# rhofield/rho-tts

Hardware: AMD Instinct MI355X
Metric: audio-sec/wall-sec (RTF) Qwen3-TTS-1.7B batch=32 (higher is better)
Workload: dtype bf16; 1 GPU; Qwen3-TTS-1.7B bf16, batch 32/GPU, 30-s reference clone, 10-word sentences (44 frames each), sampling=top-k 50 T 0.9, seeded synthetic weights; value counts delivered (post-processed) audio; global_batch=32, parallelism=dp1

## Files before the change

### rho_tts_amd/csrc/attention.hip

```cpp
#include "kernels.h"

namespace {

typedef __attribute__((ext_vector_type(4))) unsigned u4_t;

template <int D, int REP, bool FUSED, int NW, bool LO = false>
__global__ __launch_bounds__(NW * 64) void k_attention(const float* __restrict__ q, int heads, int kv_heads,
                                                   const int32_t* __restrict__ row_slot, const int32_t* __restrict__ row_pos,
                                                   int pos_add, int window, bf16_t* __restrict__ kc, bf16_t* __restrict__ vc,
                                                   int max_pos, bf16_t* __restrict__ out, const float* __restrict__ qw,
                                                   const float* __restrict__ kw, float eps, const float* __restrict__ cosT,
                                                   const float* __restrict__ sinT, const int32_t* __restrict__ frame_ptr, int out_tiled, int prefix_slot,
                                                   int prefix_len, const bf16_t* __restrict__ kc_lo, const bf16_t* __restrict__ vc_lo,
                                                   float* __restrict__ out_f32, int slot_base, int pair_n) {
    constexpr int LPP = D / 8;
    constexpr int PPW = 64 / LPP;
    constexpr int U = 4;
    __shared__ float sh[NW][REP][LPP][10];
    __shared__ float sh_q[FUSED ? REP : 1][FUSED ? D : 1];
    __shared__ __attribute__((aligned(16))) bf16_t sh_kv[2][FUSED ? D : 8];
    __shared__ __attribute__((aligned(16))) bf16_t sh_kv2[2][FUSED ? D : 8];

    const int kh = blockIdx.x, row = blockIdx.y;
    const int lane = threadIdx.x & 63, w = threadIdx.x >> 6;
    const int sub = lane % LPP, pg = lane / LPP;
    constexpr int half = D / 2;
    const int width = (heads + 2 * kv_heads) * D;
    const bool act = lane < half;
    float pa = 0.f, pb = 0.f, pwa = 0.f, pwb = 0.f, pc = 0.f, psn = 0.f;
    const int l0 = act ? lane : 0;
    if (FUSED) {
        const int v0 = w < REP + 2 ? w : REP + 1;
        const int col0 = v0 < REP ? (kh * REP + v0) * D : (v0 == REP ? (heads + kh) * D : (heads + kv_heads + kh) * D);
        const float* src = q + (int64_t)row * width + col0;
        pa = src[l0];
        pb = src[l0 + half];
        const float* nw = v0 < REP ? qw : kw;
        const float* nwp = nw ? nw : src;
        pwa = nwp[l0];
        pwb = nwp[l0 + half];
    }
    const int slot = row_slot ? row_slot[row] : slot_base + row;
    const int hi = (row_pos ? row_pos[row] : 0) + pos_add + (frame_ptr ? *frame_ptr : 0);
    if (FUSED) { pc = cosT[(int64_t)hi * half + l0]; psn = sinT[(int64_t)hi * half + l0]; }
    int lo = 0;
    if (window > 0 && hi - window + 1 > 0) lo = hi - window + 1;
    const float scale = rsqrtf((float)D);
    const bool partner = FUSED && pair_n > 0 && row >= pair_n && hi >= 1;
    const int64_t base = ((int64_t)slot * kv_heads + kh) * max_pos;
    const bf16_t* kb = kc + base * D + sub * 8;
    const bf16_t* vb = vc + base * D + sub * 8;
    const int64_t pdelta = prefix_slot >= 0 ? (((int64_t)prefix_slot - slot) * kv_heads * max_pos) * D : 0;
    constexpr int STEP = NW * PPW;
    u4_t kk[U], vv[U];
    u4_t kl[LO ? U : 1], vl[LO ? U : 1];
    auto load_batch = [&](int p0, int last) {
#pragma unroll
        for (int u = 0; u < U; ++u) {
            const int p = p0 + u * STEP;
            int pc = p <= last ? p : last;
            if (pc < 0) pc = 0;
            const int64_t po = (int64_t)pc * D + (pc < prefix_len ? pdelta : 0);
            kk[u] = *reinterpret_cast<const u4_t*>(kb + po);
            vv[u] = *reinterpret_cast<const u4_t*>(vb + po);
            if (LO) {
                kl[LO ? u : 0] = *reinterpret_cast<const u4_t*>(kc_lo + base * D + sub * 8 + po);
                vl[LO ? u : 0] = *reinterpret_cast<const u4_t*>(vc_lo + base * D + sub * 8 + po);
            }
        }
    };
    const int p_first = lo + w * PPW + pg;
    constexpr int RPL = (D * 2 >= 128) ? 1 : 128 / (D * 2);
    const int pre_last = (hi / RPL) * RPL - 1;
    constexpr bool PRE = FUSED && REP <= 2;
    if (PRE) load_batch(p_first, pre_last);

    if (FUSED) {
        for (int vec = w; vec < REP + 2 + (partner ? 2 : 0); vec += NW) {
            const bool mate = vec >= REP + 2;
            const bool is_q = vec < REP, is_k = vec == REP || vec == REP + 2;
            const int col0 = is_q ? (kh * REP + vec) * D : (is_k ? (heads + kh) * D : (heads + kv_heads + kh) * D);
            const bool first = vec == w && !mate;
            const int vrow = mate ? row - pair_n : row, vpos = mate ? hi - 1 : hi;
            float a = pa, b = pb;
            if (!first && act) { a = q[(int64_t)vrow * width + col0 + lane]; b = q[(int64_t)vrow * width + col0 + lane + half]; }
            if (is_q || is_k) {
                const float* nw = is_q ? qw : kw;
                if (nw) {
                    float wa = pwa, wb = pwb;
                    if (!first && act) { wa = nw[lane]; wb = nw[lane + half]; }
                    const float ss = wave_sum_rows_f32(act ? a * a + b * b : 0.f);
                    const float inv = rsqrtf(ss / (float)D + eps);
                    if (act) { a = wa * (a * inv); b = wb * (b * inv); }
                }
                if (act) {
                    float c = pc, s = psn;
                    if (!first) { c = cosT[(int64_t)vpos * half + lane]; s = sinT[(int64_t)vpos * half + lane]; }
                    const float ra = a * c - b * s, rb = b * c + a * s;
                    a = ra; b = rb;
                }
            }
            if (act) {
                if (is_q) { sh_q[FUSED ? vec : 0][FUSED ? lane : 0] = a; sh_q[FUSED ? vec : 0][FUSED ? lane + half : 0] = b; }
                else if (mate) {
                    sh_kv2[is_k ? 0 : 1][FUSED ? lane : 0] = f32_to_bf16(a);
                    sh_kv2[is_k ? 0 : 1][FUSED ? lane + half : 0] = f32_to_bf16(b);
                } else {
                    bf16_t* o = (is_k ? kc : vc) + (((int64_t)slot * kv_heads + kh) * max_pos + hi) * D;
                    const bf16_t ra = f32_to_bf16(a), rb = f32_to_bf16(b);
                    o[lane] = ra;
                    o[lane + half] = rb;
                    sh_kv[is_k ? 0 : 1][FUSED ? lane : 0] = ra;
                    sh_kv[is_k ? 0 : 1][FUSED ? lane + half : 0] = rb;
                }
            }
        }
        __syncthreads();
    }

    float qr[REP][8];
#pragma unroll
    for (int r = 0; r < REP; ++r) {
#pragma unroll
        for (int j = 0; j < 8; ++j) {
            if (FUSED) qr[r][j] = sh_q[FUSED ? r : 0][FUSED ? sub * 8 + j : 0] * scale;
            else qr[r][j] = q[((int64_t)row * heads + kh * REP + r) * D + sub * 8 + j] * scale;
        }
    }
    float m[REP], l[REP], acc[REP][8];
#pragma unroll
    for (int r = 0; r < REP; ++r) {
        m[r] = -1e30f;
        l[r] = 0.f;
#pragma unroll
        for (int j = 0; j < 8; ++j) acc[r][j] = 0.f;
    }
    for (int p0 = p_first; p0 <= hi; p0 += STEP * U) {
        if (PRE && p0 == p_first) {
#pragma unroll
            for (int u = 0; u < U; ++u) {
                const int p = p0 + u * STEP;
                if (p == hi) {
                    kk[u] = *reinterpret_cast<const u4_t*>(&sh_kv[0][FUSED ? sub * 8 : 0]);
                    vv[u] = *reinterpret_cast<const u4_t*>(&sh_kv[1][FUSED ? sub * 8 : 0]);
                } else if (partner && p == hi - 1) {
                    kk[u] = *reinterpret_cast<const u4_t*>(&sh_kv2[0][FUSED ? sub * 8 : 0]);
                    vv[u] = *reinterpret_cast<const u4_t*>(&sh_kv2[1][FUSED ? sub * 8 : 0]);
                } else if (p > pre_last && p < hi) {
                    const int64_t po = (int64_t)p * D + (p < prefix_len ? pdelta : 0);
                    kk[u] = *reinterpret_cast<const u4_t*>(kb + po);
                    vv[u] = *reinterpret_cast<const u4_t*>(vb + po);
                }
            }
        } else {
            load_batch(p0, hi);
        }
#pragma unroll
        for (int u = 0; u < U; ++u) {
            const int p = p0 + u * NW * PPW;
            float kf[8], vf[8];
#pragma unroll
            for (int j = 0; j < 4; ++j) {
                kf[2 * j] = __uint_as_float(kk[u][j] << 16);
                kf[2 * j + 1] = __uint_as_float(kk[u][j] & 0xffff0000u);
                vf[2 * j] = __uint_as_float(vv[u][j] << 16);
                vf[2 * j + 1] = __uint_as_float(vv[u][j] & 0xffff0000u);
                if (LO) {
                    kf[2 * j] += __uint_as_float(kl[LO ? u : 0][j] << 16);
                    kf[2 * j + 1] += __uint_as_float(kl[LO ? u : 0][j] & 0xffff0000u);
                    vf[2 * j] += __uint_as_float(vl[LO ? u : 0][j] << 16);
                    vf[2 * j + 1] += __uint_as_float(vl[LO ? u : 0][j] & 0xffff0000u);
                }
            }
#pragma unroll
            for (int r = 0; r < REP; ++r) {
                float s = 0.f;
#pragma unroll
                for (int j = 0; j < 8; ++j) s += qr[r][j] * kf[j];
                s = group_sum_f32<LPP>(s);
                if (p <= hi) {
                    const float mn = fmaxf(m[r], s);
                    const float corr = __expf(m[r] - mn), pe = __expf(s - mn);
                    l[r] = l[r] * corr + pe;
#pragma unroll
                    for (int j = 0; j < 8; ++j) acc[r][j] = acc[r][j] * corr + pe * vf[j];
                    m[r] = mn;
                }
            }
        }
    }
#pragma unroll
    for (int r = 0; r < REP; ++r) {
#pragma unroll
        for (int o = LPP; o < 64; o <<= 1) {
            const float m2 = __shfl_xor(m[r], o, 64), l2 = __shfl_xor(l[r], o, 64);
            const float mn = fmaxf(m[r], m2);
            const float c1 = __expf(m[r] - mn), c2 = __expf(m2 - mn);
            l[r] = l[r] * c1 + l2 * c2;
#pragma unroll
            for (int j = 0; j < 8; ++j) acc[r][j] = acc[r][j] * c1 + __shfl_xor(acc[r][j], o, 64) * c2;
            m[r] = mn;
        }
        if (pg == 0) {
            sh[w][r][sub][0] = m[r];
            sh[w][r][sub][1] = l[r];
#pragma unroll
            for (int j = 0; j < 8; ++j) sh[w][r][sub][2 + j] = acc[r][j];
        }
    }
    __syncthreads();
    for (int t = threadIdx.x; t < REP * LPP * 8; t += NW * 64) {
        const int j = t & 7, sb = (t >> 3) % LPP, r = t / (8 * LPP);
        float mn = -1e30f;
#pragma unroll
        for (int ww = 0; ww < NW; ++ww) mn = fmaxf(mn, sh[ww][r][sb][0]);
        float lt = 0.f, at = 0.f;
#pragma unroll
        for (int ww = 0; ww < NW; ++ww) {
            const float c = __expf(sh[ww][r][sb][0] - mn);
            lt += sh[ww][r][sb][1] * c;
            at += sh[ww][r][sb][2 + j] * c;
        }
        const int kcol = (kh * REP + r) * D + sb * 8 + j;
        const int64_t oo = out_tiled ? tile_off(row, kcol, heads * D) : (int64_t)row * heads * D + kcol;
        if (LO) out_f32[(int64_t)row * heads * D + kcol] = lt > 0.f ? at / lt : 0.f;
        else out[oo] = f32_to_bf16(lt > 0.f ? at / lt : 0.f);
    }
}

struct FusedArgs { const float *qw, *kw, *cosT, *sinT; float eps; const int32_t* frame_ptr; int out_tiled; int prefix_slot, prefix_len;
                   const bf16_t *kc_lo = nullptr, *vc_lo = nullptr; float* out_f32 = nullptr; int slot_base = 0; int pair_n = 0; };

template <int D, bool FUSED, int NW, bool LO = false>
int dispatch_rep(rt_ctx* ctx, int rep, dim3 grid, const float* q, int heads, int kv_heads, const int32_t* rs, const int32_t* rp,
                 int pos_add, int window, bf16_t* kc, bf16_t* vc, int max_pos, bf16_t* out, const FusedArgs& f) {
    switch (rep) {
        case 1: hipLaunchKernelGGL((k_attention<D, 1, FUSED, NW, LO>), grid, dim3(NW * 64), 0, ctx->stream, q, heads, kv_heads, rs, rp, pos_add, window, kc, vc, max_pos, out, f.qw, f.kw, f.eps, f.cosT, f.sinT, f.frame_ptr, f.out_tiled, f.prefix_slot, f.prefix_len, f.kc_lo, f.vc_lo, f.out_f32, f.slot_base, f.pair_n); break;
        case 2: hipLaunchKernelGGL((k_attention<D, 2, FUSED, NW, LO>), grid, dim3(NW * 64), 0, ctx->stream, q, heads, kv_heads, rs, rp, pos_add, window, kc, vc, max_pos, out, f.qw, f.kw, f.eps, f.cosT, f.sinT, f.frame_ptr, f.out_tiled, f.prefix_slot, f.prefix_len, f.kc_lo, f.vc_lo, f.out_f32, f.slot_base, f.pair_n); break;
        case 4: hipLaunchKernelGGL((k_attention<D, 4, FUSED, NW, LO>), grid, dim3(NW * 64), 0, ctx->stream, q, heads, kv_heads, rs, rp, pos_add, window, kc, vc, max_pos, out, f.qw, f.kw, f.eps, f.cosT, f.sinT, f.frame_ptr, f.out_tiled, f.prefix_slot, f.prefix_len, f.kc_lo, f.vc_lo, f.out_f32, f.slot_base, f.pair_n); break;
        default: return rt_fail(ctx, RT_ERR_UNSUPPORTED, "attention: heads/kv_heads = %d unsupported (1, 2, 4)", rep);
    }
    RT_HIP(ctx, hipGetLastError());
    return RT_OK;
}

template <bool FUSED>
int attention_any(rt_ctx* ctx, const float* q, int M, int heads, int kv_heads, int head_dim, const int32_t* row_slot, const int32_t* row_pos,
                  int pos_add, int window, const KvCache& kv, int layer, bf16_t* out, const FusedArgs& f0) {
    if (M <= 0) return RT_OK;
    FusedArgs f = f0;
    f.prefix_slot = kv.prefix_slot;
    f.prefix_len = kv.prefix_slot >= 0 ? kv.prefix_len : 0;
    if (heads % kv_heads) return rt_fail(ctx, RT_ERR_INVALID, "attention: heads %d not a multiple of kv_heads %d", heads, kv_heads);
    const int rep = heads / kv_heads;
    bf16_t* kc = kv.k + layer * kv.layer_stride();
    bf16_t* vc = kv.v + layer * kv.layer_stride();
    dim3 grid(kv_heads, M);
    if (kv.k_lo) {
        if (FUSED || !f.out_f32 || !kv.v_lo) return rt_fail(ctx, RT_ERR_INVALID, "attention: hi/lo cache needs the unfused form and a float32 output");
        f.kc_lo = kv.k_lo + layer * kv.layer_stride();
        f.vc_lo = kv.v_lo + layer * kv.layer_stride();
        switch (head_dim) {
            case 32: return dispatch_rep<32, false, 4, true>(ctx, rep, grid, q, heads, kv_heads, row_slot, row_pos, pos_add, window, kc, vc, kv.max_pos, out, f);
            case 64: return dispatch_rep<64, false, 4, true>(ctx, rep, grid, q, heads, kv_heads, row_slot, row_pos, pos_add, window, kc, vc, kv.max_pos, out, f);
            case 128: return dispatch_rep<128, false, 4, true>(ctx, rep, grid, q, heads, kv_heads, row_slot, row_pos, pos_add, window, kc, vc, kv.max_pos, out, f);
            default: return rt_fail(ctx, RT_ERR_UNSUPPORTED, "attention: head_dim %d unsupported (32, 64, 128)", head_dim);
        }
    }
    const bool wide = (FUSED || f0.frame_ptr) && M * kv_heads <= 512 && kv.max_pos > 64 && (window <= 0 || window > 256);
#define RT_ATT(DD)                                                                                                                   \
    return wide ? dispatch_rep<DD, FUSED, 16>(ctx, rep, grid, q, heads, kv_heads, row_slot, row_pos, pos_add, window, kc, vc, kv.max_pos, out, f) \
                : dispatch_rep<DD, FUSED, 4>(ctx, rep, grid, q, heads, kv_heads, row_slot, row_pos, pos_add, window, kc, vc, kv.max_pos, out, f)
    switch (head_dim) {
        case 32: RT_ATT(32);
        case 64: RT_ATT(64);
        case 128: RT_ATT(128);
        default: return rt_fail(ctx, RT_ERR_UNSUPPORTED, "attention: head_dim %d unsupported (32, 64, 128)", head_dim);
    }
#undef RT_ATT
}

}

int launch_attention(rt_ctx* ctx, const float* q, int M, int heads, int kv_heads, int head_dim, const int32_t* row_slot,
                     const int32_t* row_pos, int pos_add, int window, const KvCache& kv, int layer, bf16_t* out, const int32_t* frame_ptr, int out_tiled,
                     float* out_f32) {
    if (!frame_ptr && !out_tiled && !out_f32 && out && attention_prefill_mfma_ok(heads, kv_heads, head_dim, window, kv))
        return launch_attention_prefill_mfma(ctx, q, M, heads, kv_heads, row_slot, row_pos, pos_add, kv, layer, out);
    FusedArgs f{};
    f.frame_ptr = frame_ptr;
    f.out_tiled = out_tiled;
    f.out_f32 = out_f32;
    return attention_any<false>(ctx, q, M, heads, kv_heads, head_dim, row_slot, row_pos, pos_add, window, kv, layer, out, f);
}

int launch_attention_fused(rt_ctx* ctx, const float* qkv, int M, int heads, int kv_heads, int head_dim, const float* q_norm_w,
                           const float* k_norm_w, float eps, const float* rope_cos, const float* rope_sin, const int32_t* row_slot,
                           const int32_t* row_pos, int pos_add, int window, const KvCache& kv, int layer, bf16_t* out,
                           const int32_t* frame_ptr, int out_tiled, int slot_base, int pair_n) {
    if (!row_slot && (slot_base < 0 || slot_base + M > kv.slots))
        return rt_fail(ctx, RT_ERR_INVALID, "attention: rows %d..%d without a slot array do not fit the %d cache slots", slot_base, slot_base + M - 1, kv.slots);
    if (pair_n && (pair_n < 0 || M != 2 * pair_n || !row_slot || !row_pos || heads % kv_heads || heads / kv_heads > 2))
        return rt_fail(ctx, RT_ERR_INVALID, "attention: paired rows need M = 2 x %d rows with slot and position arrays and <= 2 query heads per kv head", pair_n);
    if (!pair_n && row_slot && row_pos && attention_mfma_ok(M, heads, kv_heads, head_dim, window, kv))
        return launch_attention_prefix_mfma(ctx, qkv, M, heads, kv_heads, q_norm_w, k_norm_w, eps, rope_cos, rope_sin, row_slot, row_pos, pos_add, kv, layer,
                                            out, frame_ptr, out_tiled);
    FusedArgs f{q_norm_w, k_norm_w, rope_cos, rope_sin, eps, frame_ptr, out_tiled, -1, 0, nullptr, nullptr, nullptr, slot_base, pair_n};
    return attention_any<true>(ctx, qkv, M, heads, kv_heads, head_dim, row_slot, row_pos, pos_add, window, kv, layer, out, f);
}
```

### rho_tts_amd/csrc/knobs.h

```cpp
#pragma once
#include "common.h"

#define RT_KNOBS(X) \
    X(0, g_skinny_variant, 0, 0, 2, "legacy skinny GEMM: 0 k_gemm_skinny, 1 k_gemm_skinny2<.,4>, 2 k_gemm_skinny2<.,8>") \
    X(100, g_decode_col, 1, 0, 1, "0 legacy 9-launch split-K decode, 1 column-owner GEMM + fused attention (5 launches per layer)") \
    X(200, g_use_graph, 1, 0, 1, "0 eager decode frames, 1 replayed from captured hipGraphs") \
    X(300, g_pred_nt, 0, 0, 1, "predictor weights: 0 cacheable loads (Infinity-Cache resident across its 15 passes), 1 non-temporal") \
    X(400, g_decode_lanes, 1, 1, 8, "decode lanes: groups of items decoding concurrently on their own streams (rt_generate)") \
    X(500, g_col_split, 0, 0, 4, "sub-tile split of narrow decode GEMMs: 0 automatic (col_split_for), 1 / 2 / 4 forced") \
    X(600, g_tile96, 1, 0, 1, "1: 128x96 workgroup tiles for N = 96 / 192 (codec decoder), 0: always 128x128") \
    X(700, g_col_rows64, 1, 0, 1, "1: one 64-row decode GEMM launch for the predictor's two-position pass, 0: two 32-row launches") \
    X(800, g_fuse_sample_embed, 1, 0, 1, "1: sampler + next-input embedding in one launch (predictor groups), 0: separate k_embed_rowsq") \
    X(900, g_prefill_fill, 3, 0, 99, "workgroups per CU a prefill GEMM's split-K aims for") \
    X(1000, g_xcd_order, 1, 0, 1, "1: tiled GEMMs run a row tile's column tiles back to back on one XCD") \
    X(1100, g_final_conv, 1, 0, 1, "the codec decoder's last conv: 1 its own LDS-window kernel, 0 a one-column GEMM") \
    X(1200, g_conv_win, 1, 0, 1, "1: k>1 convs on operand planes keep their input window in LDS (k_conv_win), 0: per-tap kernel") \
    X(1300, g_sync_parts, 0, 0, 1, "1: rt_generate waits for the stream after every frame part (bounds the dispatches in flight; profiling aid)") \
    X(1400, g_eos_check_every, 8, 1, 99, "frames between two host looks at the device-side end-of-sequence flags (1 = every frame)") \
    X(1500, g_attn_mfma, 0, 0, 2, "the talker's shared-prefix decode attention: 0 vector unit, 1 / 2 matrix cores with four rows / one row per workgroup (attention_mfma.hip); 1 measured " \
        "16.6 us per launch against 13.3 us for the vector-unit kernel at batch 32 / 460 prefix rows, so off") \
    X(1600, g_col_split4, 0, 0, 1, "1: the automatic split may go to quarter tiles (N <= 1024 on 256 CUs); measured 1.4 ms/step slower than half tiles") \
    X(1700, g_handover_every, 4, 1, 99, "queued items (n_items > rows): frames between two looks at the flags + row hand-overs.  Measured on the 1.7B model, 512 / 64 ragged texts on 32 " \
        "rows: 2 -> 487 / 445, 3 -> 489 / 445, 4 -> 491 / 447, 6 -> 485 / 445, 8 -> 477 / 428, 12 -> 475 / 434 audio-s/s (a hand-over costs ~1.4 ms, a waiting row 0.13 ms per frame)") \
    X(1800, g_conv_tall, 1, 0, 2, "k>1 convs of the 96- / 192-channel stages: 0 128-row tiles, 1 256-row tiles for long inputs, 2 always") \
    X(1900, g_prefill_mid, 1, 0, 3, "prompt prefills of 65..1024 rows: 0 split-K tiled kernel, 1 k_gemm_mid (no split-K slabs), 2 / 3 force its 64 / 128 tiles") \
    X(2000, g_col_max_rows, 64, 1, 64, "batches up to this many rows decode on the column-owner path.  Above 32 the talker's GEMMs take 64 rows per launch and the predictor's " \
        "two-position first pass runs as two 64-row launches: 715 audio-s/s at batch 64 against 510 at batch 32 (1.7B, bench.py --batch 64) - every weight byte serves twice the rows for " \
        "~1.4x the launch time") \
    X(2100, g_fuse_conv, 1, 0, 1, "1: a 96-channel k>1 conv and the 1x1 conv behind its activation run as one launch (launch_conv_pair); 0 switches the 192-channel pairs off as well") \
    X(2200, g_prefill_attn_mfma, 1, 0, 1, "prompt attention behind a shared voice prefix: 0 vector unit, 1 matrix cores") \
    X(2300, g_col_rows16, 0, 0, 1, "1: decode GEMM launches of <= 16 rows take the 128-VGPR MT = 1 instantiation (two workgroups per CU: decode lanes)") \
    X(2400, g_col_silu_x, 1, 0, 1, "1: gate/up GEMMs whose pairs are 1.5x the CUs run as one round of 1.5-pair workgroups, 0: one pair per workgroup (1.5 rounds)") \
    X(2600, g_conv_unroll, 1, 0, 1, "1: k = 7 convs run the tap-unrolled instantiation of k_conv_win, 0: the generic tap loop") \
    X(2700, g_frame_inc_fold, 0, 0, 1, "1: frame += 1 by the last workgroup of the frame's talker-input launch, 0: k_frame_inc (the fold measured 1-1.8 ms per step SLOWER)") \
    X(2800, g_pair_attn, 1, 0, 1, "1: two-position decode passes append both positions inside the fused attention launch, 0: k_qkv_post + k_attention") \
    X(2900, g_c2w_lean, 1, 0, 1, "1: rt_code2wav drops the third unit's unread residual-stream store and the waveform copy (the last conv writes the caller's buffer)") \
    X(3000, g_fuse_conv192, 1, 0, 1, "1: the 192-channel conv pairs fuse as well, weight fragments staged through LDS") \
    X(3100, g_pred_qkv_table, 1, 0, 1, "predictor passes 2..G-1: 1 layer 0's q/k/v row of the drawn code is copied from the table rt_model_finalize builds (by the launch " \
        "that embeds the code), 0 the layer-0 qkv GEMM launch runs (same bits either way)")

#define RT_KNOB_ARG(X) \
    X(0, g_skinny_waves_per_cu, 4, 1, 0x7fffffff, "legacy skinny GEMM: split-K is chosen so that about this many waves per CU stream weights")

#define RT_KNOB_EXTERN(base, name, def, lo, hi, doc) extern rt_knob name;
RT_KNOBS(RT_KNOB_EXTERN)
RT_KNOB_ARG(RT_KNOB_EXTERN)
#undef RT_KNOB_EXTERN
extern std::atomic<int> g_tune_epoch;
```

### rho_tts_amd/csrc/model_stack.hip

```cpp
#include "model_internal.h"

namespace rtm {

bool prof_events(rt_model* m, double bytes, hipEvent_t* a, hipEvent_t* b) {
    *a = *b = nullptr;
    if (!m->prof) return false;
    if (m->prof_used >= m->prof_ev.size()) {
        if (m->prof_ev.size() >= 400000) return false;
        hipEvent_t x, y;
        if (hipEventCreate(&x) != hipSuccess || hipEventCreate(&y) != hipSuccess) return false;
        m->prof_ev.push_back({x, y});
    }
    if (m->prof_tag.size() <= m->prof_used) m->prof_tag.resize(m->prof_used + 1);
    m->prof_tag[m->prof_used] = {(uint8_t)m->prof_class, bytes};
    auto& pr = m->prof_ev[m->prof_used++];
    *a = pr.first;
    *b = pr.second;
    m->prof_bytes += bytes;
    return true;
}

int gemm_rows(rt_model* m, const bf16_t* A, int rows, const PackedW& W, float* slabs, int* n_slabs) {
    if (rows <= 64) {
        const int S = skinny_pick_split(rows, W.N, W.K, m->ctx->n_cu);
        hipEvent_t e0, e1;
        prof_events(m, (double)W.N * W.K * 2.0, &e0, &e1);
        RT_TRY(launch_gemm_skinny(m->ctx, A, rows, W, slabs, W.N, S, e0, e1));
        *n_slabs = S;
    } else if (gemm_mid_shape_ok(W.N, W.K)) {
        const int n_chunks = (rows + 1023) / 1024, per = (rows + n_chunks - 1) / n_chunks;
        for (int r0 = 0; r0 < rows; r0 += per) {
            const int rc = std::min(per, rows - r0);
            if (rc > 64) RT_TRY(launch_gemm_mid(m->ctx, A + (size_t)r0 * W.K, rc, W, slabs + (size_t)r0 * W.N, W.N));
            else {
                return rt_fail(m->ctx, RT_ERR_STATE, "gemm_rows: %d-row chunk of a %d-row prefill", rc, rows);
            }
        }
        *n_slabs = 1;
    } else {
        const int S = skinny_pick_split(rows, W.N, W.K, m->ctx->n_cu);
        for (int r0 = 0; r0 < rows; r0 += 64) {
            const int rc = std::min(64, rows - r0);
            RT_TRY(launch_gemm_skinny(m->ctx, A + (size_t)r0 * W.K, rc, W, slabs + (size_t)r0 * W.N, W.N, S, nullptr, nullptr, (int64_t)rows * W.N));
        }
        *n_slabs = S;
    }
    return RT_OK;
}

int gemm_rows_f32(rt_model* m, const float* A, int rows, const PackedW& W, float* slabs, int* n_slabs) {
    (void)rows;
    int S = 1;
    while (S < 8 && W.K / (S * 2) >= 256 && (int64_t)S * 2 * W.N <= 32768) S *= 2;
    GemmA a; a.ptr = A; a.is_f32 = 1; a.split = 1; a.M = rows; a.Cin = W.K; a.taps = 1;
    GemmEpi e; e.out_f32 = slabs; e.ldc = W.N; e.split_k = S;
    RT_TRY(launch_gemm(m->ctx, a, W, e));
    *n_slabs = S;
    return RT_OK;
}

size_t slab_floats(const rt_stack_dims& d, int M, int n_cu) {
    const size_t widest = std::max<size_t>((size_t)2 * d.inter, (size_t)(d.heads + 2 * d.kv_heads) * d.head_dim);
    size_t need = std::max<size_t>((size_t)M * widest * (M > 64 ? 8 : 1), (size_t)64 * 32768);
    if (M > 64) {
        const int q = d.heads * d.head_dim, qkv = (d.heads + 2 * d.kv_heads) * d.head_dim;
        const int shapes[4][2] = {{qkv, d.hidden}, {d.hidden, q}, {2 * d.inter, d.hidden}, {d.hidden, d.inter}};
        for (auto& s : shapes)
            if (!gemm_mid_shape_ok(s[0], s[1]))
                need = std::max<size_t>(need, (size_t)M * s[0] * skinny_pick_split(M, s[0], s[1], n_cu));
    }
    return need;
}
int alloc_stack_ws(rt_model* m, const rt_stack_dims& d, int M, StackWs* w, bool precise) {
    if (precise) {
        RT_TRY(pool_arr(m, (size_t)M * d.hidden, &w->xn32));
        RT_TRY(pool_arr(m, (size_t)M * d.heads * d.head_dim, &w->ao32));
        RT_TRY(pool_arr(m, (size_t)M * d.inter, &w->act32));
        RT_TRY(pool_arr(m, slab_floats(d, M), &w->slabs));
        RT_TRY(pool_arr(m, (size_t)M * d.heads * d.head_dim, &w->q));
        return RT_OK;
    }
    RT_TRY(pool_arr(m, (size_t)M * d.hidden, &w->xn));
    RT_TRY(pool_arr(m, slab_floats(d, M), &w->slabs));
    RT_TRY(pool_arr(m, (size_t)M * d.heads * d.head_dim, &w->q));
    RT_TRY(pool_arr(m, (size_t)M * d.heads * d.head_dim, &w->ao));
    RT_TRY(pool_arr(m, (size_t)M * d.inter, &w->act));
    return RT_OK;
}

int stack_forward(rt_model* m, StackW& S, StackWs& w, float* x, int M, const int32_t* row_slot, const int32_t* row_pos, int pos_add,
                  bf16_t* out_bf16, float* out_f32, const int32_t* frame_ptr, bool prefix_rows) {
    rt_ctx* ctx = m->ctx;
    const rt_stack_dims& d = S.d;
    const int H = d.hidden;
    int ns = 0;
    const float* pending_scale = nullptr;
    if (w.xn32) {
        if (!S.kv.k_lo || !out_f32 || out_bf16) return rt_fail(ctx, RT_ERR_STATE, "stack_forward: precise mode needs hi/lo K/V planes and a float32 output");
        for (int i = 0; i < d.layers; ++i) {
            LayerW& L = S.L[i];
            RT_TRY(launch_add_rmsnorm(ctx, x, M, H, w.slabs, ns, nullptr, pending_scale, L.ln1, d.rms_eps, nullptr, w.xn32));
            RT_TRY(gemm_rows_f32(m, w.xn32, M, L.wqkv, w.slabs, &ns));
            RT_TRY(launch_qkv_post(ctx, w.slabs, ns, M, d.heads, d.kv_heads, d.head_dim, L.qn, L.kn, d.rms_eps, S.cos, S.sin, row_slot, row_pos,
                                   pos_add, w.q, S.kv, i, frame_ptr));
            RT_TRY(launch_attention(ctx, w.q, M, d.heads, d.kv_heads, d.head_dim, row_slot, row_pos, pos_add, S.window, S.kv, i, nullptr, frame_ptr, 0, w.ao32));
            RT_TRY(gemm_rows_f32(m, w.ao32, M, L.wo, w.slabs, &ns));
            RT_TRY(launch_add_rmsnorm(ctx, x, M, H, w.slabs, ns, nullptr, L.ls1, L.ln2, d.rms_eps, nullptr, w.xn32));
            RT_TRY(gemm_rows_f32(m, w.xn32, M, L.wgu, w.slabs, &ns));
            RT_TRY(launch_silu_mul(ctx, w.slabs, ns, M, d.inter, nullptr, w.act32));
            RT_TRY(gemm_rows_f32(m, w.act32, M, L.wd, w.slabs, &ns));
            pending_scale = L.ls2;
            if (g_sync_parts && !g_use_graph) RT_HIP(ctx, hipStreamSynchronize(ctx->stream));
        }
        RT_TRY(launch_add_rmsnorm(ctx, x, M, H, w.slabs, ns, nullptr, pending_scale, S.norm, d.rms_eps, nullptr, out_f32));
        return RT_OK;
    }
    for (int i = 0; i < d.layers; ++i) {
        LayerW& L = S.L[i];
        RT_TRY(launch_add_rmsnorm(ctx, x, M, H, w.slabs, ns, nullptr, pending_scale, L.ln1, d.rms_eps, w.xn, nullptr));
        RT_TRY(gemm_rows(m, w.xn, M, L.wqkv, w.slabs, &ns));
        RT_TRY(launch_qkv_post(ctx, w.slabs, ns, M, d.heads, d.kv_heads, d.head_dim, L.qn, L.kn, d.rms_eps, S.cos, S.sin, row_slot, row_pos,
                               pos_add, w.q, S.kv, i, frame_ptr));
        if (prefix_rows && pos_add == 0 && !frame_ptr && attention_block_prefix_ok(M, d.heads, d.kv_heads, d.head_dim, S.window, S.kv))
            RT_TRY(launch_attention_block_prefix(ctx, w.q, M, d.heads, d.kv_heads, row_slot, row_pos, S.kv, i, w.ao));
        else
            RT_TRY(launch_attention(ctx, w.q, M, d.heads, d.kv_heads, d.head_dim, row_slot, row_pos, pos_add, S.window, S.kv, i, w.ao, frame_ptr));
        RT_TRY(gemm_rows(m, w.ao, M, L.wo, w.slabs, &ns));
        RT_TRY(launch_add_rmsnorm(ctx, x, M, H, w.slabs, ns, nullptr, L.ls1, L.ln2, d.rms_eps, w.xn, nullptr));
        RT_TRY(gemm_rows(m, w.xn, M, L.wgu, w.slabs, &ns));
        RT_TRY(launch_silu_mul(ctx, w.slabs, ns, M, d.inter, w.act));
        RT_TRY(gemm_rows(m, w.act, M, L.wd, w.slabs, &ns));
        pending_scale = L.ls2;
        if (g_sync_parts && !g_use_graph) RT_HIP(ctx, hipStreamSynchronize(ctx->stream));
    }
    RT_TRY(launch_add_rmsnorm(ctx, x, M, H, w.slabs, ns, nullptr, pending_scale, S.norm, d.rms_eps, out_bf16, out_f32));
    return RT_OK;
}

int alloc_dec_ws(rt_model* m, const rt_stack_dims& d, int M, DecWs* w) {
    const size_t Mp = (size_t)(M + 31) / 32 * 32;
    RT_TRY(pool_arr(m, Mp * d.hidden, &w->xT));
    RT_TRY(pool_arr(m, Mp * d.hidden, &w->xa));
    RT_TRY(pool_arr(m, (size_t)M * d.heads * d.head_dim, &w->q));
    RT_TRY(pool_arr(m, (size_t)M * (d.heads + 2 * d.kv_heads) * d.head_dim, &w->qkv));
    RT_TRY(pool_arr(m, Mp * d.heads * d.head_dim, &w->ao));
    RT_TRY(pool_arr(m, Mp * d.inter, &w->act));
    return RT_OK;
}
int col_gemm(rt_model* m, const ColArgs& a0, const PackedW& W, bool is_predictor) {
    const int blk = g_col_rows64 ? 64 : 32;
    for (int r0 = 0; r0 < a0.M; r0 += blk) {
        ColArgs a = a0;
        a.nt = is_predictor ? g_pred_nt.load() : 1;
        a.M = std::min(blk, a0.M - r0);
        a.row_off = a0.row_off + r0;
        hipEvent_t e0, e1;
        prof_events(m, (double)W.N * W.K * 2.0, &e0, &e1);
        RT_TRY(launch_gemm_col(m->ctx, a, W, e0, e1));
    }
    return RT_OK;
}
int stack_qkv(rt_model* m, StackW& S, int layer, const bf16_t* xa, const float* rowsq, int M, float* out) {
    const rt_stack_dims& d = S.d;
    const int H = d.hidden, n_cu = m->ctx->n_cu, qw = (d.heads + 2 * d.kv_heads) * d.head_dim;
    ColArgs a;
    a.A = xa; a.post_scale = 1; a.rowsq = rowsq; a.rowsq_n = H / 16 * col_split_for(H, n_cu); a.eps = d.rms_eps; a.M = M; a.K = H;
    a.epi = COL_STORE; a.out = out; a.ldc = qw; a.split = col_split_for(qw, n_cu);
    return col_gemm(m, a, S.L[layer].wqkv, &S == &m->pred);
}
int stack_decode(rt_model* m, StackW& S, DecWs& w, float* x, float* rowsq, int M, const int32_t* row_slot, const int32_t* row_pos,
                 int pos_add, bool one_row_per_slot, const int32_t* frame_ptr, int slot_base, bool zero_pos, bool qkv0_ready) {
    rt_ctx* ctx = m->ctx;
    const rt_stack_dims& d = S.d;
    const int H = d.hidden, sp_h = col_split_for(H, ctx->n_cu), NTh = H / 16 * sp_h;
    const bool isp = &S == &m->pred;
    for (int i = 0; i < d.layers; ++i) {
        LayerW& L = S.L[i];
        const float* next_w = (i + 1 < d.layers) ? S.L[i + 1].ln1 : S.norm;
        if (i > 0 || !qkv0_ready) RT_TRY(stack_qkv(m, S, i, w.xa, rowsq, M, w.qkv));
        if (one_row_per_slot) {
            RT_TRY(launch_attention_fused(ctx, w.qkv, M, d.heads, d.kv_heads, d.head_dim, L.qn, L.kn, d.rms_eps, S.cos, S.sin, slot_base >= 0 ? nullptr : row_slot,
                                          zero_pos ? nullptr : row_pos, pos_add, S.window, S.kv, i, w.ao, frame_ptr, 1, slot_base));
        } else if (g_pair_attn && M % 2 == 0 && d.heads <= 2 * d.kv_heads && d.heads % d.kv_heads == 0 && row_slot && row_pos) {
            RT_TRY(launch_attention_fused(ctx, w.qkv, M, d.heads, d.kv_heads, d.head_dim, L.qn, L.kn, d.rms_eps, S.cos, S.sin, row_slot, row_pos, pos_add,
                                          S.window, S.kv, i, w.ao, frame_ptr, 1, -1, M / 2));
        } else {
            RT_TRY(launch_qkv_post(ctx, w.qkv, 1, M, d.heads, d.kv_heads, d.head_dim, L.qn, L.kn, d.rms_eps, S.cos, S.sin, row_slot, row_pos,
                                   pos_add, w.q, S.kv, i, frame_ptr));
            RT_TRY(launch_attention(ctx, w.q, M, d.heads, d.kv_heads, d.head_dim, row_slot, row_pos, pos_add, S.window, S.kv, i, w.ao, frame_ptr, 1));
        }
        ColArgs o;
        o.A = w.ao; o.M = M; o.K = d.heads * d.head_dim; o.epi = COL_RESID; o.out = x; o.ldc = H; o.scale = L.ls1;
        o.rowsq_out = rowsq; o.rowsq_out_n = NTh; o.next_bf16 = w.xa; o.next_norm_w = L.ln2; o.split = sp_h;
        RT_TRY(col_gemm(m, o, L.wo, isp));
        ColArgs gu;
        gu.A = w.xa; gu.post_scale = 1; gu.rowsq = rowsq; gu.rowsq_n = NTh; gu.eps = d.rms_eps; gu.M = M; gu.K = H;
        gu.epi = COL_SILU; gu.out_bf16 = w.act; gu.ldc = d.inter; gu.split = col_split_silu(2 * d.inter, ctx->n_cu);
        RT_TRY(col_gemm(m, gu, L.wgu, isp));
        ColArgs dn;
        dn.A = w.act; dn.M = M; dn.K = d.inter; dn.epi = COL_RESID; dn.out = x; dn.ldc = H; dn.scale = L.ls2;
        dn.rowsq_out = rowsq; dn.rowsq_out_n = NTh; dn.next_bf16 = w.xa; dn.next_norm_w = next_w; dn.split = sp_h;
        RT_TRY(col_gemm(m, dn, L.wd, isp));
        if (g_sync_parts && !g_use_graph) RT_HIP(ctx, hipStreamSynchronize(ctx->stream));
    }
    return RT_OK;
}
int col_head(rt_model* m, const bf16_t* xa, const float* rowsq, int rowsq_n, int row_off, int M, int K, float eps,
             const PackedW& W, const float* bias, float* out) {
    ColArgs a;
    a.A = xa; a.post_scale = 1; a.rowsq = rowsq; a.rowsq_n = rowsq_n; a.eps = eps; a.M = M; a.K = K; a.row_off = row_off;
    a.epi = COL_STORE; a.out = out - (size_t)row_off * W.N; a.ldc = W.N; a.bias = bias; a.split = col_split_for(W.N, m->ctx->n_cu);
    return col_gemm(m, a, W);
}

int alloc_text_ws(rt_model* m, int n, TextWs* w) {
    RT_TRY(pool_arr(m, (size_t)n * m->cfg.text_hidden, &w->e));
    RT_TRY(pool_arr(m, (size_t)n * m->cfg.text_hidden, &w->h1));
    RT_TRY(pool_arr(m, 1, &w->d_src));
    const GatherSrc src{TBL(m, "talker.text_embedding"), m->cfg.text_hidden};
    RT_HIP(m->ctx, hipMemcpy(w->d_src, &src, sizeof(src), hipMemcpyHostToDevice));
    return RT_OK;
}
int text_project(rt_model* m, const int32_t* d_ids, int n, float* out, const TextWs* ws) {
    rt_ctx* ctx = m->ctx;
    const rt_model_config& c = m->cfg;
    TextWs own;
    if (!ws) { RT_TRY(alloc_text_ws(m, n, &own)); ws = &own; }
    bf16_t *e = ws->e, *h1 = ws->h1;
    GatherSrc* d_src = ws->d_src;
    RT_TRY(launch_gather_sum(ctx, d_src, 1, d_ids, n, c.text_hidden, nullptr, nullptr, nullptr, nullptr, e));
    GemmA a; a.ptr = e; a.M = n; a.Cin = c.text_hidden;
    GemmEpi e1; e1.bias = VEC(m, "talker.tp_fc1_b"); e1.act = ACT_SILU; e1.out_bf16 = h1; e1.ldc = c.text_hidden;
    RT_TRY(launch_gemm(ctx, a, PW(m, "talker.tp_fc1"), e1));
    GemmA a2; a2.ptr = h1; a2.M = n; a2.Cin = c.text_hidden;
    GemmEpi e2; e2.bias = VEC(m, "talker.tp_fc2_b"); e2.out_f32 = out; e2.ldc = c.talker.hidden;
    RT_TRY(launch_gemm(ctx, a2, PW(m, "talker.tp_fc2"), e2));
    return RT_OK;
}

}
```

Measured before the change: 579.3 audio-s/s.

## Add lean uniform-batch attention loop and skip unread rows in predictor's last layer

Adds a LEAN variant of the fused decode attention kernel (head_dim 128, 2 query heads per KV head). Batch boundaries are decided uniformly per wave, so whole batches run without per-position predicates, the prefetched first batch is handled on its own, and the new-position patches become selects; explicit FMA ordering is meant to reproduce the old rounding bit for bit. Separately, in the predictor's two-position pass, the last layer's o-proj, gate-up and down GEMMs now run only for the second position's rows, since nothing reads the first position's. Both are on by default via knobs; the attention change adds template variants and depends on the hand-matched roundings being correct.

```diff
diff --git a/rho_tts_amd/csrc/attention.hip b/rho_tts_amd/csrc/attention.hip
--- a/rho_tts_amd/csrc/attention.hip
+++ b/rho_tts_amd/csrc/attention.hip
@@ -4,7 +4,7 @@
 
 typedef __attribute__((ext_vector_type(4))) unsigned u4_t;
 
-template <int D, int REP, bool FUSED, int NW, bool LO = false>
+template <int D, int REP, bool FUSED, int NW, bool LO = false, bool LEAN = false>
 __global__ __launch_bounds__(NW * 64) void k_attention(const float* __restrict__ q, int heads, int kv_heads,
                                                    const int32_t* __restrict__ row_slot, const int32_t* __restrict__ row_pos,
                                                    int pos_add, int window, bf16_t* __restrict__ kc, bf16_t* __restrict__ vc,
@@ -135,6 +135,80 @@
 #pragma unroll
         for (int j = 0; j < 8; ++j) acc[r][j] = 0.f;
     }
+    auto consume = [&](auto mode_tag, int p0) {
+#pragma clang fp contract(off)
+        constexpr int MODE = decltype(mode_tag)::value;
+#pragma unroll
+        for (int u = 0; u < U; ++u) {
+            const int p = p0 + u * STEP;
+            if (MODE != 2 || p <= hi) {
+                float kf[8], vf[8];
+#pragma unroll
+                for (int j = 0; j < 4; ++j) {
+                    kf[2 * j] = __uint_as_float(kk[u][j] << 16);
+                    kf[2 * j + 1] = __uint_as_float(kk[u][j] & 0xffff0000u);
+                    vf[2 * j] = __uint_as_float(vv[u][j] << 16);
+                    vf[2 * j + 1] = __uint_as_float(vv[u][j] & 0xffff0000u);
+                }
+                float s[REP];
+#pragma unroll
+                for (int r = 0; r < REP; ++r) {
+                    s[r] = __builtin_fmaf(qr[r][1], kf[1], __builtin_fmaf(qr[r][0], kf[0], 0.f));
+#pragma unroll
+                    for (int j = 2; j < 8; ++j) s[r] = u == 0 ? s[r] + qr[r][j] * kf[j] : __builtin_fmaf(qr[r][j], kf[j], s[r]);
+                    s[r] = group_sum_f32<LPP>(s[r]);
+                }
+                if (MODE != 1 || p <= hi) {
+#pragma unroll
+                    for (int r = 0; r < REP; ++r) {
+                        const float mn = fmaxf(m[r], s[r]);
+                        const float corr = __expf(m[r] - mn), pe = __expf(s[r] - mn);
+                        l[r] = __builtin_fmaf(l[r], corr, pe);
+#pragma unroll
+                        for (int j = 0; j < 8; ++j) {
+                            const float t = acc[r][j] * corr;
+                            acc[r][j] = (u == 2 && j >= 1 && j <= 6) ? pe * vf[j] + t : __builtin_fmaf(pe, vf[j], t);
+                        }
+                        m[r] = mn;
+                    }
+                }
+            }
+        }
+    };
+    using mode_t0 = std::integral_constant<int, 0>;
+    using mode_t1 = std::integral_constant<int, 1>;
+    using mode_t2 = std::integral_constant<int, 2>;
+    if constexpr (LEAN) {
+        static_assert(FUSED && D == 128 && REP == 2 && !LO && U == 4, "the roundings above were read off these forms only");
+        constexpr int BATCH = STEP * U;
+        static_assert(PRE && RPL == 1, "the prefetched batch and its patches as this block knows them");
+        const int off = w * PPW + pg;
+        if (lo + BATCH - 1 <= pre_last) {
+            consume(mode_t0{}, p_first);
+        } else if (p_first <= hi) {
+            const u4_t nk = *reinterpret_cast<const u4_t*>(&sh_kv[0][FUSED ? sub * 8 : 0]);
+            const u4_t nv = *reinterpret_cast<const u4_t*>(&sh_kv[1][FUSED ? sub * 8 : 0]);
+            const u4_t mk = *reinterpret_cast<const u4_t*>(&sh_kv2[0][FUSED ? sub * 8 : 0]);
+            const u4_t mv = *reinterpret_cast<const u4_t*>(&sh_kv2[1][FUSED ? sub * 8 : 0]);
+#pragma unroll
+            for (int u = 0; u < U; ++u) {
+                const int p = p_first + u * STEP;
+                const bool is_mate = partner && p == hi - 1, is_new = p == hi;
+                kk[u] = is_new ? nk : (is_mate ? mk : kk[u]);
+                vv[u] = is_new ? nv : (is_mate ? mv : vv[u]);
+            }
+            consume(mode_t2{}, p_first);
+        }
+        int b0 = lo + BATCH;
+        for (; b0 + BATCH - 1 <= hi; b0 += BATCH) {
+            load_batch(b0 + off, hi);
+            consume(mode_t0{}, b0 + off);
+        }
+        if (b0 + off <= hi) {
+            load_batch(b0 + off, hi);
+            consume(mode_t1{}, b0 + off);
+        }
+    } else {
     for (int p0 = p_first; p0 <= hi; p0 += STEP * U) {
         if (PRE && p0 == p_first) {
 #pragma unroll
@@ -189,6 +263,7 @@
             }
         }
     }
+    }
 #pragma unroll
     for (int r = 0; r < REP; ++r) {
 #pragma unroll
@@ -231,15 +306,27 @@
 struct FusedArgs { const float *qw, *kw, *cosT, *sinT; float eps; const int32_t* frame_ptr; int out_tiled; int prefix_slot, prefix_len;
                    const bf16_t *kc_lo = nullptr, *vc_lo = nullptr; float* out_f32 = nullptr; int slot_base = 0; int pair_n = 0; };
 
+template <int D, int REP, bool FUSED, int NW, bool LO, typename... A>
+void launch_forms(rt_ctx* ctx, dim3 grid, A... a) {
+    if constexpr (FUSED && D == 128 && REP == 2 && !LO) {
+        if (g_attn_lean) hipLaunchKernelGGL((k_attention<D, REP, FUSED, NW, LO, true>), grid, dim3(NW * 64), 0, ctx->stream, a...);
+        else hipLaunchKernelGGL((k_attention<D, REP, FUSED, NW, LO, false>), grid, dim3(NW * 64), 0, ctx->stream, a...);
+    } else {
+        hipLaunchKernelGGL((k_attention<D, REP, FUSED, NW, LO, false>), grid, dim3(NW * 64), 0, ctx->stream, a...);
+    }
+}
+
 template <int D, bool FUSED, int NW, bool LO = false>
 int dispatch_rep(rt_ctx* ctx, int rep, dim3 grid, const float* q, int heads, int kv_heads, const int32_t* rs, const int32_t* rp,
                  int pos_add, int window, bf16_t* kc, bf16_t* vc, int max_pos, bf16_t* out, const FusedArgs& f) {
+#define RT_ATT_REP(R) launch_forms<D, R, FUSED, NW, LO>(ctx, grid, q, heads, kv_heads, rs, rp, pos_add, window, kc, vc, max_pos, out, f.qw, f.kw, f.eps, f.cosT, f.sinT, f.frame_ptr, f.out_tiled, f.prefix_slot, f.prefix_len, f.kc_lo, f.vc_lo, f.out_f32, f.slot_base, f.pair_n)
     switch (rep) {
-        case 1: hipLaunchKernelGGL((k_attention<D, 1, FUSED, NW, LO>), grid, dim3(NW * 64), 0, ctx->stream, q, heads, kv_heads, rs, rp, pos_add, window, kc, vc, max_pos, out, f.qw, f.kw, f.eps, f.cosT, f.sinT, f.frame_ptr, f.out_tiled, f.prefix_slot, f.prefix_len, f.kc_lo, f.vc_lo, f.out_f32, f.slot_base, f.pair_n); break;
-        case 2: hipLaunchKernelGGL((k_attention<D, 2, FUSED, NW, LO>), grid, dim3(NW * 64), 0, ctx->stream, q, heads, kv_heads, rs, rp, pos_add, window, kc, vc, max_pos, out, f.qw, f.kw, f.eps, f.cosT, f.sinT, f.frame_ptr, f.out_tiled, f.prefix_slot, f.prefix_len, f.kc_lo, f.vc_lo, f.out_f32, f.slot_base, f.pair_n); break;
-        case 4: hipLaunchKernelGGL((k_attention<D, 4, FUSED, NW, LO>), grid, dim3(NW * 64), 0, ctx->stream, q, heads, kv_heads, rs, rp, pos_add, window, kc, vc, max_pos, out, f.qw, f.kw, f.eps, f.cosT, f.sinT, f.frame_ptr, f.out_tiled, f.prefix_slot, f.prefix_len, f.kc_lo, f.vc_lo, f.out_f32, f.slot_base, f.pair_n); break;
+        case 1: RT_ATT_REP(1); break;
+        case 2: RT_ATT_REP(2); break;
+        case 4: RT_ATT_REP(4); break;
         default: return rt_fail(ctx, RT_ERR_UNSUPPORTED, "attention: heads/kv_heads = %d unsupported (1, 2, 4)", rep);
     }
+#undef RT_ATT_REP
     RT_HIP(ctx, hipGetLastError());
     return RT_OK;
 }
diff --git a/rho_tts_amd/csrc/knobs.h b/rho_tts_amd/csrc/knobs.h
--- a/rho_tts_amd/csrc/knobs.h
+++ b/rho_tts_amd/csrc/knobs.h
@@ -37,7 +37,11 @@
     X(2900, g_c2w_lean, 1, 0, 1, "1: rt_code2wav drops the third unit's unread residual-stream store and the waveform copy (the last conv writes the caller's buffer)") \
     X(3000, g_fuse_conv192, 1, 0, 1, "1: the 192-channel conv pairs fuse as well, weight fragments staged through LDS") \
     X(3100, g_pred_qkv_table, 1, 0, 1, "predictor passes 2..G-1: 1 layer 0's q/k/v row of the drawn code is copied from the table rt_model_finalize builds (by the launch " \
-        "that embeds the code), 0 the layer-0 qkv GEMM launch runs (same bits either way)")
+        "that embeds the code), 0 the layer-0 qkv GEMM launch runs (same bits either way)") \
+    X(3200, g_attn_lean, 1, 0, 1, "k_attention's position loop, decode forms (fused, head_dim 128, 2 query heads per kv head): 1 batches decided on their base by the scalar unit " \
+        "(whole batches run without per-position predicates, the prefetched batch is its own block, patches are selects), 0 the per-lane loop (same bits)") \
+    X(3300, g_pair_last_half, 1, 0, 1, "the predictor's two-position pass, last layer: 1 o / gate-up / down run for the second position's rows only (nothing reads the " \
+        "first position's), 0 for both positions")
 
 #define RT_KNOB_ARG(X) \
     X(0, g_skinny_waves_per_cu, 4, 1, 0x7fffffff, "legacy skinny GEMM: split-K is chosen so that about this many waves per CU stream weights")
diff --git a/rho_tts_amd/csrc/model_stack.hip b/rho_tts_amd/csrc/model_stack.hip
--- a/rho_tts_amd/csrc/model_stack.hip
+++ b/rho_tts_amd/csrc/model_stack.hip
@@ -189,16 +189,18 @@
                                    pos_add, w.q, S.kv, i, frame_ptr));
             RT_TRY(launch_attention(ctx, w.q, M, d.heads, d.kv_heads, d.head_dim, row_slot, row_pos, pos_add, S.window, S.kv, i, w.ao, frame_ptr, 1));
         }
+        const bool half = !one_row_per_slot && g_pair_last_half && M % 2 == 0 && i == d.layers - 1;
+        const int r0 = half ? M / 2 : 0, Mr = M - r0;
         ColArgs o;
-        o.A = w.ao; o.M = M; o.K = d.heads * d.head_dim; o.epi = COL_RESID; o.out = x; o.ldc = H; o.scale = L.ls1;
+        o.A = w.ao; o.M = Mr; o.row_off = r0; o.K = d.heads * d.head_dim; o.epi = COL_RESID; o.out = x; o.ldc = H; o.scale = L.ls1;
         o.rowsq_out = rowsq; o.rowsq_out_n = NTh; o.next_bf16 = w.xa; o.next_norm_w = L.ln2; o.split = sp_h;
         RT_TRY(col_gemm(m, o, L.wo, isp));
         ColArgs gu;
-        gu.A = w.xa; gu.post_scale = 1; gu.rowsq = rowsq; gu.rowsq_n = NTh; gu.eps = d.rms_eps; gu.M = M; gu.K = H;
+        gu.A = w.xa; gu.post_scale = 1; gu.rowsq = rowsq; gu.rowsq_n = NTh; gu.eps = d.rms_eps; gu.M = Mr; gu.row_off = r0; gu.K = H;
         gu.epi = COL_SILU; gu.out_bf16 = w.act; gu.ldc = d.inter; gu.split = col_split_silu(2 * d.inter, ctx->n_cu);
         RT_TRY(col_gemm(m, gu, L.wgu, isp));
         ColArgs dn;
-        dn.A = w.act; dn.M = M; dn.K = d.inter; dn.epi = COL_RESID; dn.out = x; dn.ldc = H; dn.scale = L.ls2;
+        dn.A = w.act; dn.M = Mr; dn.row_off = r0; dn.K = d.inter; dn.epi = COL_RESID; dn.out = x; dn.ldc = H; dn.scale = L.ls2;
         dn.rowsq_out = rowsq; dn.rowsq_out_n = NTh; dn.next_bf16 = w.xa; dn.next_norm_w = next_w; dn.split = sp_h;
         RT_TRY(col_gemm(m, dn, L.wd, isp));
         if (g_sync_parts && !g_use_graph) RT_HIP(ctx, hipStreamSynchronize(ctx->stream));
```

Result: no change. 586.0 audio-s/s (median of 6 runs) (+1.2%).
